# nep-pack/NonlinearEigenproblems.jl

Hardware: AMD Instinct MI355X
Metric: eigenpairs/sec (gun SPMF iar m=100) + compute_Mlincomb GB/s (higher is better)
Workload: dtype f64 (complex128)

## Files before the change

include/nepmi355.h:

```cpp
#ifndef NEPMI355_H
#define NEPMI355_H

#include <stddef.h>
#include <stdint.h>

#ifdef __cplusplus
extern "C" {
#endif

typedef struct { double re, im; } nep_cdouble;
typedef struct nep_spmf nep_spmf;
typedef struct nep_lu nep_lu;
typedef struct nep_comm nep_comm;
typedef void* nep_stream;

#define NEP_OK 0
#define NEP_ERR_HIP -1
#define NEP_ERR_ARG -2
#define NEP_ERR_SINGULAR -3
#define NEP_ERR_BREAKDOWN -4
#define NEP_ERR_UNSUPPORTED -5
#define NEP_ERR_RETRY -6
#define NEP_ERR_NOCONV -7

// ... 260 lines not shown
                                      nep_stream stream);

int32_t nep_devprim_exclusive_sum(const uint64_t* d_in, uint64_t* d_out, int64_t n, nep_stream stream);
int32_t nep_devprim_sort_pairs(uint64_t* d_keys, uint64_t* d_vals, int64_t n, int32_t nbits, nep_stream stream);

typedef struct nep_iar nep_iar;
int32_t nep_iar_create(nep_spmf* spmf, nep_lu* lu, int64_t n, int32_t m, nep_cdouble* dV, int64_t ldv,
                       const nep_cdouble* dCtab, int64_t ldc, const int64_t* d_active, nep_cdouble* dwork3n,
                       const double* h_cabs, const nep_cdouble* h_cf, int32_t mt, nep_cdouble* dH, nep_cdouble* h_pinnedH,
                       int32_t orth_method, nep_iar** out);
int32_t nep_iar_destroy(nep_iar* s);
int32_t nep_iar_step(nep_iar* s, int32_t k, int32_t refine_steps, nep_stream stream);
int32_t nep_iar_steps(nep_iar* s, int32_t k0, int32_t count, int32_t refine_steps, nep_stream stream);
int32_t nep_iar_wait(nep_iar* s, int32_t k);
int32_t nep_iar_stream_wait(nep_iar* s, int32_t k, nep_stream stream);

int32_t nep_basis_rotate(nep_cdouble* dV, int64_t ldv, int64_t rows, int32_t m, int32_t p, const nep_cdouble* hQ, int64_t ldq,
                         int32_t carry, nep_stream stream);

typedef struct nep_arnoldi nep_arnoldi;
int32_t nep_arnoldi_create(nep_spmf* spmf, nep_lu* lu, int64_t n, int32_t maxdim, nep_cdouble* dV, int64_t ldv,
                           const nep_cdouble* d_cB, nep_cdouble* dwork_n, nep_cdouble* dS, nep_cdouble* h_pinnedS,
                           int32_t orth_method, nep_arnoldi** out);
int32_t nep_arnoldi_destroy(nep_arnoldi* s);
int32_t nep_arnoldi_steps(nep_arnoldi* s, int32_t j0, int32_t count, nep_stream stream);
int32_t nep_arnoldi_wait(nep_arnoldi* s, int32_t j);

typedef struct nep_iar_opts {
    int32_t maxit;
    int32_t check_error_every;
// ... 8 lines not shown
typedef struct nep_iar_result {
    int32_t k;
    int32_t nconv;
    int32_t nret;
    int32_t refine_plan;
    int32_t refine_hint_off;
    int32_t retry_reason;
} nep_iar_result;
typedef int32_t (*nep_fv_eval)(void* ctx, int32_t nlam, const nep_cdouble* lam, nep_cdouble* F);
int32_t nep_refine_review(int32_t umfpack_refinements, int32_t plan, int32_t final_recorded, const double* w4, int32_t hint_in,
                          int32_t out[4]);
int32_t nep_iar_run(nep_spmf* spmf, nep_lu* lu, int64_t n, const nep_iar_opts* opts, const nep_cdouble* h_v0,
                    const nep_cdouble* h_Ctab, int32_t mt, const double* h_cabs, const nep_cdouble* h_cf, const double* h_fro,
                    nep_fv_eval fv, void* ctx, nep_cdouble* h_lam, nep_cdouble* dQ, nep_cdouble* h_Q, double* h_err,
                    nep_cdouble* dV_basis, nep_iar_result* res, nep_stream stream);

int32_t nep_comm_unique_id(void* h_out128);
int32_t nep_comm_create(int32_t rank, int32_t world, const void* h_unique_id128, nep_comm** out);
int32_t nep_comm_destroy(nep_comm* c);
int32_t nep_comm_info(const nep_comm* c, int32_t out[2]);
int32_t nep_allgather_sum(nep_comm* c, const nep_cdouble* d_partial, int64_t len, nep_cdouble* d_total, nep_stream stream);
int32_t nep_sum_ranks(const nep_cdouble* d_parts, int64_t len, int32_t world, nep_cdouble* d_total, nep_stream stream);

typedef struct nep_bem nep_bem;
int32_t nep_bem_create(int64_t n, const double* h_vert, const double* h_area, int32_t gauss_order, nep_bem** out);
int32_t nep_bem_destroy(nep_bem* b);
int32_t nep_bem_info(const nep_bem* b, int64_t info[4]);
int32_t nep_bem_static(const nep_bem* b, double* d_out, int64_t ldo, nep_stream stream);
int32_t nep_bem_assemble(const nep_bem* b, int32_t nlam, const nep_cdouble* h_lam, int32_t der, nep_cdouble* dOut, int64_t ldo,
                         int64_t stride, nep_stream stream);
// ... 20 lines not shown
```

nonlineareigenproblems.jl_amd/_lib.py:

```python
import ctypes as C
import os

import numpy as np
import torch

from ._env import env_flag

_HERE = os.path.dirname(os.path.abspath(__file__))
LIB_PATH = os.path.join(_HERE, "libnepmi355.so")


class NepError(RuntimeError):
    def __init__(self, status, msg):
        super().__init__("libnepmi355 status %d: %s" % (status, msg))
        self.status = status


NEP_OK, NEP_ERR_HIP, NEP_ERR_ARG, NEP_ERR_SINGULAR, NEP_ERR_BREAKDOWN, NEP_ERR_UNSUPPORTED = 0, -1, -2, -3, -4, -5
NEP_ERR_RETRY, NEP_ERR_NOCONV = -6, -7


def _load():
    from . import build
    if build.needs_build():
# ... 140 lines not shown
    "nep_iar_create": [c_vp, c_vp, c_i64, c_i32, c_vp, c_i64, c_vp, c_i64, c_vp, c_vp, c_vp, c_vp, c_i32, c_vp, c_vp, c_i32, P(c_vp)],
    "nep_iar_destroy": [c_vp],
    "nep_lu_refac_create": [c_vp, c_i64, c_vp, c_vp, c_vp, c_vp, c_vp, c_vp, c_vp, c_vp, c_vp],
    "nep_lu_refac_destroy": [c_vp],
    "nep_lu_refac_info": [c_vp, c_vp],
    "nep_lu_refac_wide_info": [c_vp, c_vp],
    "nep_lu_refac_hash": [c_vp, c_vp],
    "nep_lu_factor_dev": [c_vp, c_vp, c_i32, C.c_double, c_vp, c_vp, c_vp, c_vp],
    "nep_lu_refac_analyze": [c_i64, c_vp, c_vp, c_vp, c_vp, c_vp, c_vp, c_vp, c_vp, c_vp],
    "nep_lu_factor_dev_batch": [c_vp, c_i32, c_vp, c_i32, C.c_double, c_vp, c_vp, c_vp, c_vp],
    "nep_lu_factor_dev_batch_terms": [c_vp, c_i32, c_vp, c_i32, c_vp, c_i32, C.c_double, c_vp, c_vp, c_vp],
    "nep_iar_step": [c_vp, c_i32, c_i32, c_vp],
    "nep_iar_steps": [c_vp, c_i32, c_i32, c_i32, c_vp],
    "nep_iar_wait": [c_vp, c_i32],
    "nep_iar_stream_wait": [c_vp, c_i32, c_vp],
    "nep_basis_rotate": [c_vp, c_i64, c_i64, c_i32, c_i32, c_vp, c_i64, c_i32, c_vp],
    "nep_arnoldi_create": [c_vp, c_vp, c_i64, c_i32, c_vp, c_i64, c_vp, c_vp, c_vp, c_vp, c_i32, P(c_vp)],
    "nep_arnoldi_destroy": [c_vp],
    "nep_arnoldi_steps": [c_vp, c_i32, c_i32, c_vp],
    "nep_arnoldi_wait": [c_vp, c_i32],
    "nep_devprim_exclusive_sum": [c_vp, c_vp, c_i64, c_vp],
    "nep_devprim_sort_pairs": [c_vp, c_vp, c_i64, c_i32, c_vp],
    "nep_refine_review": [c_i32, c_i32, c_i32, c_vp, c_i32, c_vp],
    "nep_iar_run": [c_vp, c_vp, c_i64, c_vp, c_vp, c_vp, c_i32, c_vp, c_vp, c_vp, c_vp, c_vp, c_vp, c_vp, c_vp, c_vp, c_vp, c_vp, c_vp],
    "nep_hess_eig_worksize": [c_i32, P(c_i64)],
    "nep_hess_eigvals_dev": [c_i32, c_vp, c_i64, c_vp, c_vp, c_vp, c_vp],
    "nep_hess_eigvecs_dev": [c_i32, c_vp, c_vp, c_i64, c_vp, c_vp, c_vp],
    "nep_hess_eigvals_batch_dev": [c_i32, c_i32, c_i32, c_vp, c_i64, c_vp, c_i64, c_vp, c_i64, c_vp, c_i64, c_vp],
    "nep_hess_eigvecs_batch_dev": [c_i32, c_i32, c_i32, c_vp, c_i64, c_vp, c_i64, c_i64, c_vp, c_i64, c_vp, c_i64, c_vp],
    "nep_comm_unique_id": [c_vp],
    "nep_comm_create": [c_i32, c_i32, c_vp, P(c_vp)],
    "nep_comm_destroy": [c_vp],
    "nep_comm_info": [c_vp, P(c_i32)],
    "nep_allgather_sum": [c_vp, c_vp, c_i64, c_vp, c_vp],
    "nep_sum_ranks": [c_vp, c_i64, c_i32, c_vp, c_vp],
    "nep_iar_shift_scale": [c_i64, c_i32, c_vp, c_vp, c_vp],
    "nep_rk_bw": [c_i64, c_i32, c_vp, c_vp, c_vp, c_vp],
    "nep_discretize_polygon": [c_i32, c_vp, c_i32, c_vp],
    "nep_block_recur": [c_i64, c_i32, c_vp, c_vp, c_vp, c_vp, c_vp],
# ... 59 lines not shown
```

nonlineareigenproblems.jl_amd/csrc/driver.hip:

```cpp
#include "common.h"
#include <vector>
#include <stdlib.h>
#include <time.h>

struct nep_iar {
    nep_spmf* spmf; nep_lu* lu;
    int64_t n, ldv; int32_t m, mt;
    cplx* dV; const cplx* dCtab; int64_t ldc; const int64_t* d_active;
    cplx* dz; cplx* dW;
    std::vector<double> cabs; std::vector<nep_cdouble> cf;
    cplx* dH; nep_cdouble* hH;
    double* d_cabs; cplx* d_ccf;
    cplx* hH_dev;
    int32_t method;
    std::vector<hipEvent_t> ev;
    hipEvent_t e_upload = nullptr; bool upload_waited = false;
    hipStream_t last = nullptr;
    bool no_events = false;
    std::vector<hipGraphExec_t> graphs;
    cplx* dWT = nullptr; int32_t wt_for = 0;
};

extern "C" {

int32_t nep_iar_create(nep_spmf* spmf, nep_lu* lu, int64_t n, int32_t m, nep_cdouble* dV, int64_t ldv,
                       const nep_cdouble* dCtab, int64_t ldc, const int64_t* d_active, nep_cdouble* dwork3n,
                       const double* h_cabs, const nep_cdouble* h_cf, int32_t mt, nep_cdouble* dH, nep_cdouble* h_pinnedH,
                       int32_t orth_method, nep_iar** out) {
    ARGCHK(out != nullptr);
    *out = nullptr;
    ARGCHK(spmf && lu && dV && dCtab && dwork3n && dH && h_pinnedH);
    ARGCHK(n > 0 && m >= 1 && ldv >= n * (int64_t)(m + 1) && ldc >= m && mt >= 1 && (orth_method == 0 || orth_method == 1));
    nep_iar* s = new nep_iar();
// ... 91 lines not shown
        rc = nep_iar_shift_scale(n, k, (const nep_cdouble*)col, (nep_cdouble*)vv, stream);
        if (rc) return rc;
    }
    cplx* mirror = s->hH_dev ? s->hH_dev + (int64_t)(k - 1) * (s->m + 4) : nullptr;
    if (s->dWT && k < s->m) {
        rc = nep_orth_dev_iar_next((const nep_cdouble*)s->dV, s->ldv, n, k, s->d_active, (nep_cdouble*)vv, (nep_cdouble*)hrow, s->method,
                                   (nep_cdouble*)mirror, k + 4, (const nep_cdouble*)s->dCtab, s->ldc, s->mt,
                                   (nep_cdouble*)s->dWT, (nep_cdouble*)(vv + s->ldv + n), stream);
        if (!rc) s->wt_for = k + 1;
    } else
        rc = nep_orth_dev_mirror((const nep_cdouble*)s->dV, s->ldv, n * (int64_t)(k + 1), k, s->d_active, (nep_cdouble*)vv,
                                 (nep_cdouble*)hrow, s->method, (nep_cdouble*)mirror, k + 4, stream);
    if (rc) return rc;
    if (!mirror)
        HIPCHK(hipMemcpyAsync(s->hH + (int64_t)(k - 1) * (s->m + 4), hrow, (size_t)(k + 4) * sizeof(cplx), hipMemcpyDeviceToHost, st));
    if (s->no_events) return NEP_OK;
    if (!s->ev[k]) HIPCHK(hipEventCreateWithFlags(&s->ev[k], hipEventDisableTiming | hipEventBlockingSync));
    HIPCHK(hipEventRecord(s->ev[k], st));
    return NEP_OK;
}

int32_t nep_iar_steps(nep_iar* s, int32_t k0, int32_t count, int32_t refine_steps, nep_stream stream) {
    ARGCHK(s && count >= 1);
    for (int32_t k = k0; k < k0 + count; ++k) {
        int rc = nep_iar_step(s, k, refine_steps, stream);
        if (rc) return rc;
    }
    return NEP_OK;
}

int32_t nep_iar_steps_graph(nep_iar* s, int32_t k0, int32_t count, int32_t refine_steps, nep_stream stream, int32_t* captured) {
    ARGCHK(s && count >= 1);
    if (captured) *captured = 0;
// ... 8 lines not shown
        hipGraph_t g = nullptr;
        hipError_t e = hipStreamEndCapture(st, &g);
        hipGraphExec_t ge = nullptr;
        if (!rc && e == hipSuccess && g && hipGraphInstantiate(&ge, g, nullptr, nullptr, 0) == hipSuccess && ge) {
            if (hipGraphLaunch(ge, st) == hipSuccess) { s->graphs.push_back(ge); ok = true; }
            else (void)hipGraphExecDestroy(ge);
        }
        if (g) (void)hipGraphDestroy(g);
        if (!ok) (void)hipGetLastError();
    } else (void)hipGetLastError();
    if (!ok) {
        s->wt_for = wt_for0; s->upload_waited = waited0; s->last = last0;
        return nep_iar_steps(s, k0, count, refine_steps, stream);
    }
    for (int32_t k = k0; k < k0 + count; ++k) {
        if (!s->ev[k]) HIPCHK(hipEventCreateWithFlags(&s->ev[k], hipEventDisableTiming | hipEventBlockingSync));
        HIPCHK(hipEventRecord(s->ev[k], st));
    }
    if (captured) *captured = 1;
    return NEP_OK;
}

int32_t nep_iar_wait(nep_iar* s, int32_t k) {
    ARGCHK(s && k >= 1 && k <= s->m && s->ev[k]);
    for (;;) {
        const hipError_t e = hipEventQuery(s->ev[k]);
        if (e == hipSuccess) return NEP_OK;
        if (e != hipErrorNotReady) HIPCHK(e);
        struct timespec ts = {0, 20000};
        nanosleep(&ts, nullptr);
    }
}

int32_t nep_iar_stream_wait(nep_iar* s, int32_t k, nep_stream stream) {
    ARGCHK(s && k >= 1 && k <= s->m && s->ev[k]);
    HIPCHK(hipStreamWaitEvent(as_stream(stream), s->ev[k], 0));
    return NEP_OK;
}

}
```

nonlineareigenproblems.jl_amd/csrc/iar_run.hip:

```cpp
#include "common.h"
#include <algorithm>
#include <deque>
#include <map>
#include <mutex>
#include <vector>
#include <math.h>
#include <time.h>

extern "C" {
int32_t nep_iar_create(nep_spmf* spmf, nep_lu* lu, int64_t n, int32_t m, nep_cdouble* dV, int64_t ldv, const nep_cdouble* dCtab,
                       int64_t ldc, const int64_t* d_active, nep_cdouble* dwork3n, const double* h_cabs, const nep_cdouble* h_cf,
                       int32_t mt, nep_cdouble* dH, nep_cdouble* h_pinnedH, int32_t orth_method, nep_iar** out);
int32_t nep_iar_steps_graph(nep_iar* s, int32_t k0, int32_t count, int32_t refine_steps, nep_stream stream, int32_t* captured);
}

namespace {

constexpr double EPS = 2.220446049250313e-16;

__global__ void k_iar_active(int64_t* act, int64_t n, int m1) {
    const int j = blockIdx.x * blockDim.x + threadIdx.x;
    if (j < m1) act[j] = (int64_t)(j + 1) * n;
}
__global__ void k_iar_start(cplx* __restrict__ V, const cplx* __restrict__ v, double inv, int64_t n) {
    const int64_t i = (int64_t)blockIdx.x * blockDim.x + threadIdx.x;
    if (i < n) V[i] = cmake(v[i].x * inv, v[i].y * inv);
}

constexpr int64_t ZSLACK = 8192;
__global__ __launch_bounds__(256) void k_iar_zero_slack(cplx* __restrict__ V, int64_t ldv, int64_t n, int m1) {
    const int j = blockIdx.y;
    const int64_t a = (int64_t)(j + 1) * n;
    const int64_t r = a + (int64_t)blockIdx.x * 256 + threadIdx.x;
// ... 160 lines not shown
    std::vector<hipEvent_t> ev_pool;
    std::vector<double> s_lam; std::vector<int> s_idx; cplx* s_QT = nullptr; int s_kq = 0; int conv = 0; int k_checked = 0;
    std::vector<double> s_err;
    double* h_err = nullptr;
    int retry = 0;

    hipEvent_t event() {
        if (!ev_pool.empty()) { hipEvent_t e = ev_pool.back(); ev_pool.pop_back(); return e; }
        hipEvent_t e = nullptr;
        if (hipEventCreateWithFlags(&e, hipEventDisableTiming) != hipSuccess) { (void)hipGetLastError(); return nullptr; }
        return e;
    }
    void done(hipEvent_t e) { if (e) ev_pool.push_back(e); }

    int fail_kind = 0, fail_at = 0;
    int fill_H(int kk) {
        for (int j = 1; j <= kk; ++j) {
            if (filled[j]) continue;
            if (fail_at == j && (fail_kind == 1 || fail_kind == 2)) {
                retry = fail_kind; nep_set_error("nep_iar_run: injected miss of kind %d at step %d", fail_kind, j); return NEP_ERR_RETRY;
            }
            const cplx* row = a.Hpin + (int64_t)(j - 1) * (m + 4);
            const int flags = (int)row[j + 1].y;
            if (flags & 2) { nep_set_error("orthogonalisation breakdown in step %d: ||w|| = %g", j, row[j].x); return NEP_ERR_BREAKDOWN; }
            if ((flags & 1) && o.orth_method == 0) { retry = 2; nep_set_error("nep_iar_run: step %d wanted another DGKS pass", j); return NEP_ERR_RETRY; }
            if (ref.umf > 0) {
                const int plan = plans[j];
                const bool final_rec = !((plan & 0x100) && (j % 8) != 0);
                if (!ref.review((const double*)(row + j + 2), plan & 0xff, final_rec)) {
                    retry = 1; nep_set_error("nep_iar_run: the refinement record of step %d asks for more sweeps than were taken", j);
                    return NEP_ERR_RETRY;
                }
            }
            filled[j] = 1;
        }
        return NEP_OK;
    }
    ~Run() {
        if (step) (void)nep_iar_destroy(step);
        if (V && own_V) nep_pool_free_on(V, st, true);
        if (s_QT) nep_pool_free_on(s_QT, rs.check, true);
        for (hipEvent_t e : ev_pool) (void)hipEventDestroy(e);
        if (have_arena) arena_return(a);
    }
};

}

extern "C" {

int32_t nep_refine_review(int32_t umfpack_refinements, int32_t plan, int32_t final_recorded, const double* w4, int32_t hint_in,
                          int32_t out[4]) {
    ARGCHK(w4 && out && plan >= 0 && plan <= 3 && umfpack_refinements >= 0);
    Refine r; r.umf = umfpack_refinements; r.hint = hint_in;
    const bool ok = r.review(w4, plan, final_recorded != 0);
    out[0] = ok ? 1 : 0; out[1] = r.recorded; out[2] = r.hint; out[3] = r.hint_off ? 1 : 0;
    return NEP_OK;
}

int32_t nep_iar_run(nep_spmf* spmf, nep_lu* lu, int64_t n, const nep_iar_opts* opts, const nep_cdouble* h_v0,
                    const nep_cdouble* h_Ctab, int32_t mt, const double* h_cabs, const nep_cdouble* h_cf, const double* h_fro,
                    nep_fv_eval fv, void* ctx, nep_cdouble* h_lam, nep_cdouble* dQ, nep_cdouble* h_Q, double* h_err,
                    nep_cdouble* dV_basis, nep_iar_result* res, nep_stream stream) {
    ARGCHK(spmf && lu && opts && h_v0 && h_Ctab && fv && h_lam && res);
    ARGCHK(n > 0 && mt >= 1 && opts->maxit >= 1 && opts->check_error_every >= 1);
    ARGCHK(opts->orth_method == 0 || opts->orth_method == 1);
    ARGCHK(opts->errmeasure == 0 || (opts->errmeasure == 1 && h_fro));
    ARGCHK(opts->umfpack_refinements <= 0 || (h_cabs && h_cf));
    memset(res, 0, sizeof(*res));
    res->refine_plan = -1;
    struct timespec t_e_; clock_gettime(CLOCK_MONOTONIC, &t_e_);
    const double t_entry = t_e_.tv_sec * 1e3 + t_e_.tv_nsec * 1e-6;
    const int32_t m = opts->maxit;
    if (m > 128) { nep_set_error("nep_iar_run: maxit = %d exceeds the device eigen-decomposition's limit 128", m); return NEP_ERR_UNSUPPORTED; }
    const int BMAX = std::max(1, nep_env_int("NEP_IAR_EIG_BATCH", 16));
    const int LASTB = std::max(1, nep_env_int("NEP_IAR_EIG_LAST", 8));
    const double T100 = nep_env_double("NEP_IAR_EIG_MS100", 3.3);
    const double TSTEP = 0.35;
    const int cee = opts->check_error_every;
    const double neigs = opts->neigs;
    const bool unthrottled = isinf(neigs) && neigs > 0;

    Run R; R.spmf = spmf; R.lu = lu; R.n = n; R.o = *opts; R.fv = fv; R.ctx = ctx; R.h_fro = h_fro; R.st = as_stream(stream);
    R.m = m; R.mt = mt; R.ldv = n * (int64_t)(m + 1); R.h_err = h_err;
    int rc = run_streams(R.st, &R.rs); if (rc) return rc;
    rc = arena_acquire(n, m, mt, BMAX, &R.a); if (rc) return rc;
    R.have_arena = true;
    Arena& a = R.a;
    hipStream_t st = R.st, cst = R.rs.check, est = R.rs.eig;
    R.ref.umf = opts->umfpack_refinements > 0 ? opts->umfpack_refinements : 0;
    R.ref.hint = (opts->refine_hint >= 0 && nep_env_int("NEP_REFINE_HINT", 1) != 0) ? opts->refine_hint : -1;
    R.filled.assign(m + 1, 0); R.plans.assign(m + 1, 0);
    if (const char* fa = getenv("NEP_IAR_RUN_FAIL_AT")) { if (sscanf(fa, "%d:%d", &R.fail_kind, &R.fail_at) != 2) R.fail_kind = R.fail_at = 0; }
    if (h_err) for (int64_t i = 0; i < (int64_t)m * m; ++i) h_err[i] = NAN;

    if (dV_basis) { R.V = (cplx*)dV_basis; R.own_V = false; }
// ... 14 lines not shown
    }
    hipLaunchKernelGGL(k_iar_start, dim3((unsigned)((n + 255) / 256)), dim3(256), 0, st, R.V, (const cplx*)a.v0, 1.0 / sqrt(nrm2), n);
    hipLaunchKernelGGL(k_iar_active, dim3((unsigned)((m + 1 + 63) / 64)), dim3(64), 0, st, a.active, n, m + 1);
    HIPCHK(hipMemsetAsync(a.Hdev, 0, (size_t)m * (m + 4) * 16, st));
    LAUNCHCHK();
    memset(a.Hpin, 0, (size_t)m * (m + 4) * 16);
    memset(a.wpin, 0, (size_t)m * (m + 2) * 16);
    {
        static thread_local PinnedRing ring;
        rc = ring.upload(a.Ctab, h_Ctab, (size_t)m * mt * 16, st); if (rc) return rc;
    }
    rc = nep_iar_create(spmf, lu, n, m, (nep_cdouble*)R.V, R.ldv, (const nep_cdouble*)a.Ctab, m, a.active, (nep_cdouble*)a.work3n,
                        R.ref.umf > 0 ? h_cabs : nullptr, R.ref.umf > 0 ? h_cf : nullptr, mt, (nep_cdouble*)a.Hdev,
                        (nep_cdouble*)a.Hpin, opts->orth_method, &R.step);
    if (rc) return rc;

    std::vector<char> plan_end(m + 2, 0);
    if (unthrottled) {
        std::vector<int> allk;
        for (int kk = 1; kk <= m; ++kk) if (kk % cee == 0 || kk == m) allk.push_back(kk);
        int e_ = (int)allk.size(); int size = std::min(LASTB, e_);
        while (e_ > 0) {
            plan_end[allk[e_ - 1]] = 1; e_ -= size;
            if (e_ > 0) {
                const double q = allk[e_ - 1] / 100.0;
                size = (int)std::min<double>(std::min(BMAX, e_), std::max(1.0, ceil(2.0 * T100 * q * q / (TSTEP * cee))));
            }
        }
    }
    const bool trace = getenv("NEP_IAR_RUN_TRACE") != nullptr;
    auto now = []() { struct timespec t; clock_gettime(CLOCK_MONOTONIC, &t); return t.tv_sec * 1e3 + t.tv_nsec * 1e-6; };
    double t_fv = 0;
    std::deque<int> pendA; std::deque<Batch> stA; std::deque<Check> stC;
    int slots = unthrottled ? m + 1 : std::max(BMAX, 4);
    const int CHUNK = unthrottled ? 8 : 4;
    const int P = std::min(256, std::max(1, 3072 / mt));
    int k = 1; bool done = false; int status = NEP_OK;
    const bool use_graph = nep_env_flag("NEP_IAR_GRAPH");
    int n_graph = 0;
    auto finished = [&]() { return R.conv >= neigs; };

    auto batch_ready = [&]() -> int {
        if (pendA.empty()) return 0;
        int cnt = 1;
        while (cnt < (int)pendA.size() && cnt < BMAX && pendA[cnt] - pendA[cnt - 1] == pendA[1] - pendA[0] && !(unthrottled && plan_end[pendA[cnt - 1]])) ++cnt;
        if (!unthrottled || plan_end[pendA[cnt - 1]] || cnt >= BMAX || done) return cnt;
        return 0;
    };
    auto launch_batch = [&](int count) -> int {
        Batch b;
        for (int i = 0; i < count; ++i) { b.kcs.push_back(pendA.front()); pendA.pop_front(); }
        const int k0 = b.kcs[0], nb = count; b.kmax = b.kcs.back();
        const int kstep = nb > 1 ? b.kcs[1] - k0 : 0;
        int r = nep_iar_stream_wait(R.step, b.kmax, (nep_stream)est); if (r) return r;
        cplx* wrow = a.wdev + (int64_t)(k0 - 1) * (m + 2);
        cplx* mrow = a.wpin + (int64_t)(k0 - 1) * (m + 2);
        r = nep_hess_eigvals_batch_dev(nb, k0, kstep, (const nep_cdouble*)a.Hdev, m + 4, (nep_cdouble*)wrow, (int64_t)kstep * (m + 2),
                                       a.eigwork, a.wsz, (nep_cdouble*)mrow, (int64_t)kstep * (m + 2), (nep_stream)est);
        if (r) return r;
        b.evW = R.event(); if (!b.evW) return NEP_ERR_HIP;
        HIPCHK(hipEventRecord(b.evW, est));
        void* pz = nullptr;
        r = nep_pool_alloc(&pz, (size_t)nb * b.kmax * b.kmax * 16); if (r) return r;
        b.Zb = (cplx*)pz;
        r = nep_hess_eigvecs_batch_dev(nb, k0, kstep, (nep_cdouble*)wrow, (int64_t)kstep * (m + 2), (nep_cdouble*)b.Zb, b.kmax,
                                       (int64_t)b.kmax * b.kmax, a.eigwork, a.wsz, (nep_cdouble*)mrow, (int64_t)kstep * (m + 2), (nep_stream)est);
        if (r) { nep_pool_free_on(b.Zb, est, true); return r; }
        b.evZ = R.event(); if (!b.evZ) return NEP_ERR_HIP;
        HIPCHK(hipEventRecord(b.evZ, est));
        stA.push_back(b);
        return NEP_OK;
    };
    auto launch_check = [&](const Batch& b, int bi, bool first_of_batch) -> int {
        const int kc = b.kcs[bi];
        int r = R.fill_H(kc); if (r) return r;
        const cplx* w = a.wpin + (int64_t)(kc - 1) * (m + 2);
        if (w[kc].x != 0.0 || (R.fail_kind == 3 && R.fail_at == kc)) { R.retry = 3; nep_set_error("nep_iar_run: the QR iteration of step %d gave up", kc); return NEP_ERR_RETRY; }
        Check c; c.kc = kc; c.lam.resize(2 * (size_t)kc); c.F.resize(2 * (size_t)mt * kc);
        const double sr = R.o.sigma.re, si = R.o.sigma.im, gr = R.o.gamma.re, gi = R.o.gamma.im;
        for (int s = 0; s < kc; ++s) {
            const double dr = w[s].x, di = w[s].y, den = dr * dr + di * di;
            c.lam[2 * s] = sr + (gr * dr + gi * di) / den;
            c.lam[2 * s + 1] = si + (gi * dr - gr * di) / den;
        }
        const double tf0 = trace ? now() : 0.0;
        const int32_t frc = R.fv(R.ctx, kc, (const nep_cdouble*)c.lam.data(), (nep_cdouble*)c.F.data());
        if (trace) t_fv += now() - tf0;
        if (frc != 0) {
            nep_set_error("nep_iar_run: the f_t(lambda) callback failed in step %d", kc); return NEP_ERR_ARG;
        }
        if (first_of_batch) HIPCHK(hipStreamWaitEvent(cst, b.evZ, 0));
        void* pq = nullptr;
        r = nep_pool_alloc(&pq, (size_t)n * kc * 16); if (r) return r;
        c.QT = (cplx*)pq;
        r = nep_gemm_ts_dev((const nep_cdouble*)R.V, R.ldv, n, kc, (const nep_cdouble*)(b.Zb + (int64_t)bi * b.kmax * b.kmax), b.kmax, 0, kc,
                            (nep_cdouble*)c.QT, kc, 1, (nep_stream)cst);
        double* d_out = a.d_norms + (int64_t)(kc - 1) * 2 * m;
        if (!r) r = nep_resid_batch_dev(spmf, kc, (const nep_cdouble*)c.F.data(), (const nep_cdouble*)c.QT, kc, d_out, (nep_stream)cst);
        if (r) { nep_pool_free_on(c.QT, cst, true); return r; }
        HIPCHK(hipMemcpyAsync(a.npin + (int64_t)(kc - 1) * 2 * m, d_out, (size_t)2 * kc * 8, hipMemcpyDeviceToHost, cst));
        c.ev = R.event(); if (!c.ev) return NEP_ERR_HIP;
        HIPCHK(hipEventRecord(c.ev, cst));
        if (bi == (int)b.kcs.size() - 1) c.Zb_owner = b.Zb;
        stC.push_back(std::move(c));
        return NEP_OK;
    };
// ... 42 lines not shown
        return NEP_OK;
    };
    auto drop_check = [&](Check& c) {
        if (c.QT) nep_pool_free_on(c.QT, cst, true);
        if (c.Zb_owner) nep_pool_free_on(c.Zb_owner, cst, true);
        R.done(c.ev);
    };
    auto drop_batch = [&](Batch& b) {
        if (b.Zb) nep_pool_free_on(b.Zb, est, true);
        R.done(b.evW); R.done(b.evZ);
    };

    hipEvent_t te0 = nullptr, te1 = nullptr; bool te1_rec = false;
    if (trace) { (void)hipEventCreate(&te0); (void)hipEventCreate(&te1); (void)hipEventRecord(te0, st); }
    const double t_loop = now();
    double tt_steps = 0, tt_A = 0, tt_B = 0, tt_C = 0, tt_sleep = 0, t_enq_done = 0; double tq = 0;
    while (status == NEP_OK) {
        bool progressed = false;
        tq = now();
        if (!done) {
            if (k <= m && !finished()) {
                int nb = 0;
                while (nb < CHUNK && k + nb <= m) {
                    const bool due = ((k + nb) % cee == 0) || (k + nb == m);
                    if (due) { if (slots <= 0) break; --slots; }
                    ++nb;
                }
                if (nb > 0) {
                    int plan = R.ref.plan();
                    if (plan > 0 && R.ref.settled()) plan |= 0x100;
                    if (use_graph && k > 1) { int32_t cap = 0; status = nep_iar_steps_graph(R.step, k, nb, plan, stream, &cap); n_graph += cap; }
                    else status = nep_iar_steps(R.step, k, nb, plan, stream);
                    if (status) break;
                    for (int kk = k; kk < k + nb; ++kk) {
                        R.plans[kk] = plan;
                        if (kk % cee == 0 || kk == m) pendA.push_back(kk);
                    }
                    k += nb; progressed = true;
                }
            } else done = true;
            if (k > m) { if (!done && trace) { t_enq_done = now() - t_loop; if (te1 && !te1_rec) { (void)hipEventRecord(te1, st); te1_rec = true; } } done = true; }
        }
        if (trace) { const double t = now(); tt_steps += t - tq; tq = t; }
        while (!finished()) {
            const int cnt = batch_ready();
            if (!cnt) break;
            status = launch_batch(cnt); progressed = true;
            if (status) break;
        }
        if (status) break;
        if (trace) { const double t = now(); tt_A += t - tq; tq = t; }
        while (!stA.empty() && !finished() && ev_done(stA.front().evW)) {
            progressed = true;
            Batch b = stA.front(); stA.pop_front();
            for (int bi = 0; bi < (int)b.kcs.size() && status == NEP_OK; ++bi) {
                status = launch_check(b, bi, bi == 0);
// ... 22 lines not shown
        if (done && pendA.empty() && stA.empty() && stC.empty()) break;
        if (!progressed) { struct timespec ts = {0, 20000}; nanosleep(&ts, nullptr); if (trace) { const double t = now(); tt_sleep += t - tq; tq = t; } }
    }
    if (trace)
        fprintf(stderr, "nep_iar_run trace (ms): set-up %.2f | loop %.2f: steps %.2f (all enqueued at %.2f) A %.2f B %.2f (callback %.2f) C %.2f sleep %.2f\n",
                t_loop - t_entry, now() - t_loop, tt_steps, t_enq_done, tt_A, tt_B, t_fv, tt_C, tt_sleep);
    if (trace && use_graph) fprintf(stderr, "nep_iar_run: %d chunks went out as hipGraphs\n", n_graph);
    if (trace && te0 && te1 && te1_rec) {
        float ms_ = 0.0f;
        if (hipEventSynchronize(te1) == hipSuccess && hipEventElapsedTime(&ms_, te0, te1) == hipSuccess)
            fprintf(stderr, "nep_iar_run: the recurrence's %d steps took %.2f ms on the device\n", m, ms_);
        (void)hipGetLastError();
    }
    if (te0) (void)hipEventDestroy(te0);
    if (te1) (void)hipEventDestroy(te1);
    while (!stA.empty()) { drop_batch(stA.front()); stA.pop_front(); }
    while (!stC.empty()) { drop_check(stC.front()); stC.pop_front(); }
    (void)hipStreamSynchronize(est);
    (void)hipStreamSynchronize(cst);
    res->retry_reason = R.retry;
    res->refine_plan = R.ref.hint_off ? -1 : (R.ref.recorded >= 0 ? R.ref.recorded : R.ref.hint);
    res->refine_hint_off = R.ref.hint_off ? 1 : 0;
    if (status || !unthrottled) (void)hipStreamSynchronize(st);
    if (status) return status;

    int nret = (int)(R.s_lam.size() / 2);
    const bool noconv = (R.conv < neigs) && !unthrottled;
    if (!noconv) nret = std::min(nret, R.conv);
    res->k = R.k_checked > 0 ? R.k_checked : k - 1;
    res->nconv = R.conv; res->nret = nret;
    for (int s = 0; s < nret; ++s) { h_lam[s].re = R.s_lam[2 * s]; h_lam[s].im = R.s_lam[2 * s + 1]; }
    if (nret > 0 && (dQ || h_Q) && R.s_QT) {
        cplx* dst = (cplx*)dQ; void* tmp = nullptr;
        if (!dst) { rc = nep_pool_alloc(&tmp, (size_t)n * nret * 16); if (rc) return rc; dst = (cplx*)tmp; }
        std::vector<int32_t> cols(R.s_idx.begin(), R.s_idx.begin() + nret);
        rc = nep_rowmajor_to_colmajor(n, R.s_kq, (const nep_cdouble*)R.s_QT, R.s_kq, cols.data(), nret, (nep_cdouble*)dst, n, (nep_stream)cst);
        if (!rc && h_Q) {
            if (hipMemcpyAsync(h_Q, dst, (size_t)n * nret * 16, hipMemcpyDeviceToHost, cst) != hipSuccess) rc = NEP_ERR_HIP;
        }
        if (hipStreamSynchronize(cst) != hipSuccess && !rc) rc = NEP_ERR_HIP;
        if (tmp) nep_pool_free(tmp);
        if (rc) { if (rc == NEP_ERR_HIP) nep_set_error("nep_iar_run: returning the eigenvector block failed"); return rc; }
    }
    if (noconv) { nep_set_error("Number of iterations exceeded. maxit=%d.", m); return NEP_ERR_NOCONV; }
    return NEP_OK;
}

}
```

nonlineareigenproblems.jl_amd/iar.py:

```python
import contextlib
import ctypes as _C
import queue
import threading
import time
from collections import deque
from concurrent.futures import ThreadPoolExecutor
from typing import NamedTuple

import numpy as np
import torch

from . import dense, _hosteig
from ._affinity import cpu_budget
from ._env import env_flag, env_float, env_int, env_str
from ._lib import (lib, check, c_vp, c_i32, hptr, cdouble, NepError, IarOpts, IarResult, FV_EVAL, NEP_ERR_BREAKDOWN, NEP_ERR_RETRY,
                   NEP_ERR_NOCONV)
from ._ritzchecks import RitzChecks
from ._streams import _check_stream, _eig_streams
from .errmeasure import (DefaultErrmeasure, ResidualErrmeasure, StandardSPMFErrmeasure, estimate_errors, estimate_errors_async)
from .exceptions import NoConvergenceException
from .linsolvers import DefaultLinSolverCreator, FactorizeLinSolver, create_linsolver
from .nep import CDT, AbstractSPMF, pure_spmf, to_host, to_host_cm, stream_ptr

EPS = np.finfo(float).eps
# ... 116 lines not shown

def _route(f):
    if not f.staged():
        return "sync"
    if not f.native():
        return "async"
    dev_eig = f.m <= dense.HESS_EIG_KMAX and env_str("NEP_IAR_EIG", "dev") != "host"
    if (f.native_run and f.native_err and dev_eig and env_str("NEP_IAR_NATIVE_RUN", "1") != "0"
            and not any(env_flag(e) for e in ("NEP_IAR_TRACE", "NEP_IAR_ONE_STREAM", "NEP_IAR_PASSES"))):
        return "run"
    if env_flag("NEP_IAR_ONE_STREAM") or not f.batch_async:
        return "async"
    return "step+deveig" if dev_eig else "step+hosteig"


def _iar_native_run(nep, M0inv, orthmethod, m, tol, neigs, errkind, sigma, gamma, v, check_error_every, errhist, return_device):
    n = nep.size(1)
    fv = nep.get_fv(); mt = len(fv)
    alpha = gamma ** np.arange(m + 1); alpha[0] = 0
    tab = nep.derivative_table(sigma, m)
    Ctab = np.asfortranarray((alpha[1:m + 1] / np.arange(1, m + 1))[:, None] * tab["fD"][1:m + 1, :], dtype=np.complex128)
    v0 = np.ascontiguousarray(v, dtype=np.complex128)
    rc_ = M0inv.refine_coefficients() if M0inv.umfpack_refinements > 0 else None
    if M0inv.umfpack_refinements > 0 and rc_ is None:
        return None
    o = IarOpts(m, int(check_error_every), dense._orth_code(orthmethod), int(max(0, M0inv.umfpack_refinements)), errkind[0],
                -1, float(tol), float(neigs), cdouble(sigma.real, sigma.imag), cdouble(gamma.real, gamma.imag))
    res = IarResult()

    def fv_eval(ctx, nlam, lam_p, F_p):
        try:
            la = np.frombuffer((_C.c_double * (2 * nlam)).from_address(lam_p), dtype=np.complex128)
            F = np.frombuffer((_C.c_double * (2 * nlam * mt)).from_address(F_p), dtype=np.complex128).reshape(nlam, mt)
            for t, f in enumerate(fv):
                F[:, t] = f.values(la)
            return 0
        except Exception:
            import traceback
            traceback.print_exc()
            return 1
    cb = FV_EVAL(fv_eval)
    ldv = n * (m + 1)
    V = torch.empty((m + 1, ldv), dtype=CDT, device="cuda")
    Qd = torch.empty((m, n), dtype=CDT, device="cuda") if return_device else None
    Qh = None if return_device else torch.empty((m, n), dtype=CDT, pin_memory=True)
    lam = np.zeros(m, dtype=np.complex128)
    err = np.full((m, m), np.nan, order="F")
    st = M0inv.refine.native_run(o, res, lambda: lib.nep_iar_run(
        nep.dev.h, M0inv.lu.h, n, _C.addressof(o), hptr(v0), hptr(Ctab), mt,
        hptr(rc_[0]) if rc_ else None, hptr(rc_[1]) if rc_ else None, hptr(errkind[1]) if errkind[1] is not None else None,
        _C.cast(cb, c_vp), None, hptr(lam), c_vp(Qd.data_ptr()) if Qd is not None else None,
        c_vp(Qh.data_ptr()) if Qh is not None else None, hptr(err), c_vp(V.data_ptr()), _C.addressof(res), stream_ptr()))
    if st == NEP_ERR_RETRY:
        if res.retry_reason == 1:
            raise _RefinementMiss(0)
        if res.retry_reason == 2:
            raise _OrthPassMiss(0)
        raise _NativeRunMiss(res.retry_reason)
    if st not in (0, NEP_ERR_NOCONV):
        check(st)
    iar.native_runs += 1
    iar.last_route = "run"
    k = int(res.k); nret = int(res.nret)
    M0inv.refine.solves += k
    if errhist is not None:
        for kc in range(1, k + 1):
            if kc % check_error_every == 0 or kc == m:
# ... 19 lines not shown
        linsolvercreator = DefaultLinSolverCreator()
    if errmeasure is None:
        errmeasure = DefaultErrmeasure(nep)
    if v is None:
        v = np.random.randn(n)
    errkind = _native_errmeasure(errmeasure, nep)
    f = _Facts(m=m, orth=dense._orth_code(orthmethod), dev_lu=True, native_err=errkind is not None,
               spmf_dev=_plain_spmf(nep) and type(nep).resid_norms is AbstractSPMF.resid_norms and hasattr(nep, "dev"),
               batch_async=hasattr(errmeasure, "batch_async"), timed=timers is not None, proj_solve=bool(proj_solve),
               native_run=_native_run, native_step=_native_step, force_sync=_force_sync)
    M0inv = None
    if _route(f) == "run":
        M0inv = create_linsolver(linsolvercreator, nep, sigma)
        if _device_lu(M0inv):
            out = _iar_native_run(nep, M0inv, orthmethod, m, tol, neigs, errkind, sigma, gamma, v, check_error_every, errhist,
                                  return_device)
            if out is not None:
                return out
    s = _State(t_entry, nep, orthmethod, m, linsolvercreator, M0inv, tol, neigs, errmeasure, sigma, gamma, v, check_error_every,
               proj_solve, errhist, timers, inner_solver_method, f.staged())
    f = f._replace(native_run=False, spmf_dev=_plain_spmf(nep) and "Cdev" in s.tab, dev_lu=_device_lu(s.M0inv))
    if f.native() and not s.create_native_step():
        f = f._replace(dev_lu=False)
    route = iar.last_route = _route(f)
    s.start(route)
    try:
        k = {"sync": _run_sync, "async": _run_async}.get(route, _run_steps)(s)
    finally:
        s.close()
    k = s.checks.k_checked if s.checks.k_checked > 0 else k - 1
    lam, Q = s.checks.finish(k, maxit, "Try to change the inner_solver_method for better performance.",
# ... 489 lines not shown
```

Before: 1434.

## Skip per-step error history and thin IAR events when unthrottled without history

When neigs is infinite and no error history or logger is requested, the native IAR run sets the check cadence to the final step only. It also records completion events only at chunk boundaries, and the host no longer allocates the error matrix. Row review and refinement checks are decoupled from the eigenvalue checks and done lazily: a lag gate polls step readiness with a non-blocking query before enqueuing further chunks, and the rest is reviewed once enqueueing finishes. The aim is to cut Hessenberg eigen decompositions, residual checks, event records and host syncs, at the cost of more complex control flow and bounded enqueue-ahead.

```diff
diff --git a/include/nepmi355.h b/include/nepmi355.h
--- a/include/nepmi355.h
+++ b/include/nepmi355.h
@@ -298,6 +298,8 @@
 int32_t nep_iar_steps(nep_iar* s, int32_t k0, int32_t count, int32_t refine_steps, nep_stream stream);
 int32_t nep_iar_wait(nep_iar* s, int32_t k);
 int32_t nep_iar_stream_wait(nep_iar* s, int32_t k, nep_stream stream);
+int32_t nep_iar_ready(nep_iar* s, int32_t k, int32_t* ready);
+int32_t nep_iar_event_mask(nep_iar* s, const uint8_t* mask);
 
 int32_t nep_basis_rotate(nep_cdouble* dV, int64_t ldv, int64_t rows, int32_t m, int32_t p, const nep_cdouble* hQ, int64_t ldq,
                          int32_t carry, nep_stream stream);
@@ -336,6 +338,7 @@
                     const nep_cdouble* h_Ctab, int32_t mt, const double* h_cabs, const nep_cdouble* h_cf, const double* h_fro,
                     nep_fv_eval fv, void* ctx, nep_cdouble* h_lam, nep_cdouble* dQ, nep_cdouble* h_Q, double* h_err,
                     nep_cdouble* dV_basis, nep_iar_result* res, nep_stream stream);
+int32_t nep_iar_run_stats(int32_t out[4]);
 
 int32_t nep_comm_unique_id(void* h_out128);
 int32_t nep_comm_create(int32_t rank, int32_t world, const void* h_unique_id128, nep_comm** out);
diff --git a/nonlineareigenproblems.jl_amd/_lib.py b/nonlineareigenproblems.jl_amd/_lib.py
--- a/nonlineareigenproblems.jl_amd/_lib.py
+++ b/nonlineareigenproblems.jl_amd/_lib.py
@@ -178,6 +178,8 @@
     "nep_iar_steps": [c_vp, c_i32, c_i32, c_i32, c_vp],
     "nep_iar_wait": [c_vp, c_i32],
     "nep_iar_stream_wait": [c_vp, c_i32, c_vp],
+    "nep_iar_ready": [c_vp, c_i32, P(c_i32)],
+    "nep_iar_event_mask": [c_vp, c_vp],
     "nep_basis_rotate": [c_vp, c_i64, c_i64, c_i32, c_i32, c_vp, c_i64, c_i32, c_vp],
     "nep_arnoldi_create": [c_vp, c_vp, c_i64, c_i32, c_vp, c_i64, c_vp, c_vp, c_vp, c_vp, c_i32, P(c_vp)],
     "nep_arnoldi_destroy": [c_vp],
@@ -187,6 +189,7 @@
     "nep_devprim_sort_pairs": [c_vp, c_vp, c_i64, c_i32, c_vp],
     "nep_refine_review": [c_i32, c_i32, c_i32, c_vp, c_i32, c_vp],
     "nep_iar_run": [c_vp, c_vp, c_i64, c_vp, c_vp, c_vp, c_i32, c_vp, c_vp, c_vp, c_vp, c_vp, c_vp, c_vp, c_vp, c_vp, c_vp, c_vp, c_vp],
+    "nep_iar_run_stats": [P(c_i32)],
     "nep_hess_eig_worksize": [c_i32, P(c_i64)],
     "nep_hess_eigvals_dev": [c_i32, c_vp, c_i64, c_vp, c_vp, c_vp, c_vp],
     "nep_hess_eigvecs_dev": [c_i32, c_vp, c_vp, c_i64, c_vp, c_vp, c_vp],
diff --git a/nonlineareigenproblems.jl_amd/csrc/driver.hip b/nonlineareigenproblems.jl_amd/csrc/driver.hip
--- a/nonlineareigenproblems.jl_amd/csrc/driver.hip
+++ b/nonlineareigenproblems.jl_amd/csrc/driver.hip
@@ -17,6 +17,8 @@
     hipEvent_t e_upload = nullptr; bool upload_waited = false;
     hipStream_t last = nullptr;
     bool no_events = false;
+    std::vector<uint8_t> ev_mask;
+    int32_t n_ev = 0;
     std::vector<hipGraphExec_t> graphs;
     cplx* dWT = nullptr; int32_t wt_for = 0;
 };
@@ -138,9 +140,23 @@
     if (rc) return rc;
     if (!mirror)
         HIPCHK(hipMemcpyAsync(s->hH + (int64_t)(k - 1) * (s->m + 4), hrow, (size_t)(k + 4) * sizeof(cplx), hipMemcpyDeviceToHost, st));
-    if (s->no_events) return NEP_OK;
+    if (s->no_events || (!s->ev_mask.empty() && !s->ev_mask[k])) return NEP_OK;
     if (!s->ev[k]) HIPCHK(hipEventCreateWithFlags(&s->ev[k], hipEventDisableTiming | hipEventBlockingSync));
     HIPCHK(hipEventRecord(s->ev[k], st));
+    ++s->n_ev;
+    return NEP_OK;
+}
+
+int32_t nep_iar_event_mask(nep_iar* s, const uint8_t* mask) {
+    ARGCHK(s != nullptr);
+    ARGCHK(s->last == nullptr && s->n_ev == 0);
+    if (mask) s->ev_mask.assign(mask, mask + s->m + 1); else s->ev_mask.clear();
+    return NEP_OK;
+}
+
+int32_t nep_iar_events_recorded(const nep_iar* s, int32_t* out) {
+    ARGCHK(s && out);
+    *out = s->n_ev;
     return NEP_OK;
 }
 
@@ -179,8 +195,10 @@
         return nep_iar_steps(s, k0, count, refine_steps, stream);
     }
     for (int32_t k = k0; k < k0 + count; ++k) {
+        if (!s->ev_mask.empty() && !s->ev_mask[k]) continue;
         if (!s->ev[k]) HIPCHK(hipEventCreateWithFlags(&s->ev[k], hipEventDisableTiming | hipEventBlockingSync));
         HIPCHK(hipEventRecord(s->ev[k], st));
+        ++s->n_ev;
     }
     if (captured) *captured = 1;
     return NEP_OK;
@@ -197,6 +215,15 @@
     }
 }
 
+int32_t nep_iar_ready(nep_iar* s, int32_t k, int32_t* ready) {
+    ARGCHK(s && ready && k >= 1 && k <= s->m && s->ev[k]);
+    const hipError_t e = hipEventQuery(s->ev[k]);
+    if (e == hipErrorNotReady) (void)hipGetLastError();
+    else if (e != hipSuccess) HIPCHK(e);
+    *ready = e == hipSuccess ? 1 : 0;
+    return NEP_OK;
+}
+
 int32_t nep_iar_stream_wait(nep_iar* s, int32_t k, nep_stream stream) {
     ARGCHK(s && k >= 1 && k <= s->m && s->ev[k]);
     HIPCHK(hipStreamWaitEvent(as_stream(stream), s->ev[k], 0));
diff --git a/nonlineareigenproblems.jl_amd/csrc/iar_run.hip b/nonlineareigenproblems.jl_amd/csrc/iar_run.hip
--- a/nonlineareigenproblems.jl_amd/csrc/iar_run.hip
+++ b/nonlineareigenproblems.jl_amd/csrc/iar_run.hip
@@ -12,11 +12,14 @@
                        int64_t ldc, const int64_t* d_active, nep_cdouble* dwork3n, const double* h_cabs, const nep_cdouble* h_cf,
                        int32_t mt, nep_cdouble* dH, nep_cdouble* h_pinnedH, int32_t orth_method, nep_iar** out);
 int32_t nep_iar_steps_graph(nep_iar* s, int32_t k0, int32_t count, int32_t refine_steps, nep_stream stream, int32_t* captured);
+int32_t nep_iar_events_recorded(const nep_iar* s, int32_t* out);
 }
 
 namespace {
 
 constexpr double EPS = 2.220446049250313e-16;
+
+thread_local int32_t g_run_stats[4] = {0, 0, 0, 0};
 
 __global__ void k_iar_active(int64_t* act, int64_t n, int m1) {
     const int j = blockIdx.x * blockDim.x + threadIdx.x;
@@ -207,16 +210,28 @@
     void done(hipEvent_t e) { if (e) ev_pool.push_back(e); }
 
     int fail_kind = 0, fail_at = 0;
-    int fill_H(int kk) {
-        for (int j = 1; j <= kk; ++j) {
-            if (filled[j]) continue;
-            if (fail_at == j && (fail_kind == 1 || fail_kind == 2)) {
+    int flagged = 0, reviewed = 0;
+    int check_flags(int kk) {
+        for (int j = flagged + 1; j <= kk; ++j) {
+            if (fail_at == j && fail_kind == 2) {
                 retry = fail_kind; nep_set_error("nep_iar_run: injected miss of kind %d at step %d", fail_kind, j); return NEP_ERR_RETRY;
             }
             const cplx* row = a.Hpin + (int64_t)(j - 1) * (m + 4);
             const int flags = (int)row[j + 1].y;
             if (flags & 2) { nep_set_error("orthogonalisation breakdown in step %d: ||w|| = %g", j, row[j].x); return NEP_ERR_BREAKDOWN; }
             if ((flags & 1) && o.orth_method == 0) { retry = 2; nep_set_error("nep_iar_run: step %d wanted another DGKS pass", j); return NEP_ERR_RETRY; }
+            flagged = j;
+        }
+        return NEP_OK;
+    }
+    int fill_H(int kk) {
+        const int rf = check_flags(kk); if (rf) return rf;
+        for (int j = 1; j <= kk; ++j) {
+            if (filled[j]) continue;
+            if (fail_at == j && fail_kind == 1) {
+                retry = fail_kind; nep_set_error("nep_iar_run: injected miss of kind %d at step %d", fail_kind, j); return NEP_ERR_RETRY;
+            }
+            const cplx* row = a.Hpin + (int64_t)(j - 1) * (m + 4);
             if (ref.umf > 0) {
                 const int plan = plans[j];
                 const bool final_rec = !((plan & 0x100) && (j % 8) != 0);
@@ -225,12 +240,13 @@
                     return NEP_ERR_RETRY;
                 }
             }
-            filled[j] = 1;
-        }
+            filled[j] = 1; ++g_run_stats[3];
+        }
+        reviewed = std::max(reviewed, kk);
         return NEP_OK;
     }
     ~Run() {
-        if (step) (void)nep_iar_destroy(step);
+        if (step) { (void)nep_iar_events_recorded(step, &g_run_stats[2]); (void)nep_iar_destroy(step); }
         if (V && own_V) nep_pool_free_on(V, st, true);
         if (s_QT) nep_pool_free_on(s_QT, rs.check, true);
         for (hipEvent_t e : ev_pool) (void)hipEventDestroy(e);
@@ -255,6 +271,7 @@
                     const nep_cdouble* h_Ctab, int32_t mt, const double* h_cabs, const nep_cdouble* h_cf, const double* h_fro,
                     nep_fv_eval fv, void* ctx, nep_cdouble* h_lam, nep_cdouble* dQ, nep_cdouble* h_Q, double* h_err,
                     nep_cdouble* dV_basis, nep_iar_result* res, nep_stream stream) {
+    for (int i = 0; i < 4; ++i) g_run_stats[i] = 0;
     ARGCHK(spmf && lu && opts && h_v0 && h_Ctab && fv && h_lam && res);
     ARGCHK(n > 0 && mt >= 1 && opts->maxit >= 1 && opts->check_error_every >= 1);
     ARGCHK(opts->orth_method == 0 || opts->orth_method == 1);
@@ -270,9 +287,13 @@
     const int LASTB = std::max(1, nep_env_int("NEP_IAR_EIG_LAST", 8));
     const double T100 = nep_env_double("NEP_IAR_EIG_MS100", 3.3);
     const double TSTEP = 0.35;
-    const int cee = opts->check_error_every;
     const double neigs = opts->neigs;
     const bool unthrottled = isinf(neigs) && neigs > 0;
+    const bool nohist = unthrottled && !h_err;
+    const int cee = nohist ? m : opts->check_error_every;
+    auto due_at = [&](int kk) { return kk % cee == 0 || kk == m; };
+    const int CHUNK = unthrottled ? 8 : 4;
+    const int LAG = 3 * CHUNK;
 
     Run R; R.spmf = spmf; R.lu = lu; R.n = n; R.o = *opts; R.fv = fv; R.ctx = ctx; R.h_fro = h_fro; R.st = as_stream(stream);
     R.m = m; R.mt = mt; R.ldv = n * (int64_t)(m + 1); R.h_err = h_err;
@@ -317,11 +338,16 @@
                         R.ref.umf > 0 ? h_cabs : nullptr, R.ref.umf > 0 ? h_cf : nullptr, mt, (nep_cdouble*)a.Hdev,
                         (nep_cdouble*)a.Hpin, opts->orth_method, &R.step);
     if (rc) return rc;
+    if (nohist) {
+        std::vector<uint8_t> mask(m + 1, 0);
+        for (int kk = 1; kk <= m; ++kk) mask[kk] = (kk % CHUNK == 0 || kk == m) ? 1 : 0;
+        rc = nep_iar_event_mask(R.step, mask.data()); if (rc) return rc;
+    }
 
     std::vector<char> plan_end(m + 2, 0);
     if (unthrottled) {
         std::vector<int> allk;
-        for (int kk = 1; kk <= m; ++kk) if (kk % cee == 0 || kk == m) allk.push_back(kk);
+        for (int kk = 1; kk <= m; ++kk) if (due_at(kk)) allk.push_back(kk);
         int e_ = (int)allk.size(); int size = std::min(LASTB, e_);
         while (e_ > 0) {
             plan_end[allk[e_ - 1]] = 1; e_ -= size;
@@ -336,7 +362,6 @@
     double t_fv = 0;
     std::deque<int> pendA; std::deque<Batch> stA; std::deque<Check> stC;
     int slots = unthrottled ? m + 1 : std::max(BMAX, 4);
-    const int CHUNK = unthrottled ? 8 : 4;
     const int P = std::min(256, std::max(1, 3072 / mt));
     int k = 1; bool done = false; int status = NEP_OK;
     const bool use_graph = nep_env_flag("NEP_IAR_GRAPH");
@@ -361,6 +386,7 @@
         r = nep_hess_eigvals_batch_dev(nb, k0, kstep, (const nep_cdouble*)a.Hdev, m + 4, (nep_cdouble*)wrow, (int64_t)kstep * (m + 2),
                                        a.eigwork, a.wsz, (nep_cdouble*)mrow, (int64_t)kstep * (m + 2), (nep_stream)est);
         if (r) return r;
+        g_run_stats[0] += nb;
         b.evW = R.event(); if (!b.evW) return NEP_ERR_HIP;
         HIPCHK(hipEventRecord(b.evW, est));
         void* pz = nullptr;
@@ -376,7 +402,7 @@
     };
     auto launch_check = [&](const Batch& b, int bi, bool first_of_batch) -> int {
         const int kc = b.kcs[bi];
-        int r = R.fill_H(kc); if (r) return r;
+        int r = R.check_flags(kc); if (r) return r;
         const cplx* w = a.wpin + (int64_t)(kc - 1) * (m + 2);
         if (w[kc].x != 0.0 || (R.fail_kind == 3 && R.fail_at == kc)) { R.retry = 3; nep_set_error("nep_iar_run: the QR iteration of step %d gave up", kc); return NEP_ERR_RETRY; }
         Check c; c.kc = kc; c.lam.resize(2 * (size_t)kc); c.F.resize(2 * (size_t)mt * kc);
@@ -393,6 +419,7 @@
             nep_set_error("nep_iar_run: the f_t(lambda) callback failed in step %d", kc); return NEP_ERR_ARG;
         }
         if (first_of_batch) HIPCHK(hipStreamWaitEvent(cst, b.evZ, 0));
+        ++g_run_stats[1];
         void* pq = nullptr;
         r = nep_pool_alloc(&pq, (size_t)n * kc * 16); if (r) return r;
         c.QT = (cplx*)pq;
@@ -465,16 +492,23 @@
     hipEvent_t te0 = nullptr, te1 = nullptr; bool te1_rec = false;
     if (trace) { (void)hipEventCreate(&te0); (void)hipEventCreate(&te1); (void)hipEventRecord(te0, st); }
     const double t_loop = now();
-    double tt_steps = 0, tt_A = 0, tt_B = 0, tt_C = 0, tt_sleep = 0, t_enq_done = 0; double tq = 0;
+    double tt_steps = 0, tt_A = 0, tt_B = 0, tt_C = 0, tt_sleep = 0, t_enq_done = 0, t_m_done = 0; double tq = 0;
     while (status == NEP_OK) {
         bool progressed = false;
         tq = now();
         if (!done) {
             if (k <= m && !finished()) {
+                const int g = (k - 1) / CHUNK * CHUNK - LAG;
+                bool gate_open = true;
+                if (g >= 1 && !R.filled[g]) {
+                    int32_t ready = 0;
+                    status = nep_iar_ready(R.step, g, &ready); if (status) break;
+                    if (ready) { status = R.fill_H(g); if (status) break; }
+                    else gate_open = false;
+                }
                 int nb = 0;
-                while (nb < CHUNK && k + nb <= m) {
-                    const bool due = ((k + nb) % cee == 0) || (k + nb == m);
-                    if (due) { if (slots <= 0) break; --slots; }
+                while (gate_open && nb < CHUNK && k + nb <= m && !(nb > 0 && (k + nb - 1) % CHUNK == 0)) {
+                    if (due_at(k + nb)) { if (slots <= 0) break; --slots; }
                     ++nb;
                 }
                 if (nb > 0) {
@@ -485,12 +519,23 @@
                     if (status) break;
                     for (int kk = k; kk < k + nb; ++kk) {
                         R.plans[kk] = plan;
-                        if (kk % cee == 0 || kk == m) pendA.push_back(kk);
+                        if (due_at(kk)) pendA.push_back(kk);
                     }
                     k += nb; progressed = true;
                 }
             } else done = true;
             if (k > m) { if (!done && trace) { t_enq_done = now() - t_loop; if (te1 && !te1_rec) { (void)hipEventRecord(te1, st); te1_rec = true; } } done = true; }
+        }
+        if (k > m && !finished()) {
+            while (R.reviewed < m) {
+                const int g = std::min((R.reviewed / CHUNK + 1) * CHUNK, m);
+                int32_t ready = 0;
+                status = nep_iar_ready(R.step, g, &ready); if (status || !ready) break;
+                status = R.fill_H(g); if (status) break;
+                progressed = true;
+                if (g == m && trace) t_m_done = now();
+            }
+            if (status) break;
         }
         if (trace) { const double t = now(); tt_steps += t - tq; tq = t; }
         while (!finished()) {
@@ -543,6 +588,7 @@
     }
     if (te0) (void)hipEventDestroy(te0);
     if (te1) (void)hipEventDestroy(te1);
+    if (status == NEP_OK && R.k_checked > 0) status = R.fill_H(R.k_checked);
     while (!stA.empty()) { drop_batch(stA.front()); stA.pop_front(); }
     while (!stC.empty()) { drop_check(stC.front()); stC.pop_front(); }
     (void)hipStreamSynchronize(est);
@@ -571,8 +617,17 @@
         if (tmp) nep_pool_free(tmp);
         if (rc) { if (rc == NEP_ERR_HIP) nep_set_error("nep_iar_run: returning the eigenvector block failed"); return rc; }
     }
+    if (trace && t_m_done > 0)
+        fprintf(stderr, "nep_iar_run: %.2f ms from the arrival of step %d's row to the return (%d decompositions, %d checks)\n",
+                now() - t_m_done, m, g_run_stats[0], g_run_stats[1]);
     if (noconv) { nep_set_error("Number of iterations exceeded. maxit=%d.", m); return NEP_ERR_NOCONV; }
     return NEP_OK;
 }
 
-}
+int32_t nep_iar_run_stats(int32_t out[4]) {
+    ARGCHK(out != nullptr);
+    for (int i = 0; i < 4; ++i) out[i] = g_run_stats[i];
+    return NEP_OK;
+}
+
+}
diff --git a/nonlineareigenproblems.jl_amd/iar.py b/nonlineareigenproblems.jl_amd/iar.py
--- a/nonlineareigenproblems.jl_amd/iar.py
+++ b/nonlineareigenproblems.jl_amd/iar.py
@@ -154,7 +154,12 @@
     return "step+deveig" if dev_eig else "step+hosteig"
 
 
-def _iar_native_run(nep, M0inv, orthmethod, m, tol, neigs, errkind, sigma, gamma, v, check_error_every, errhist, return_device):
+def _native_run_keeps_history(errhist, neigs, logger):
+    return errhist is not None or bool(logger) or not (np.isinf(neigs) and neigs > 0)
+
+
+def _iar_native_run(nep, M0inv, orthmethod, m, tol, neigs, errkind, sigma, gamma, v, check_error_every, errhist, return_device,
+                    logger=0):
     n = nep.size(1)
     fv = nep.get_fv(); mt = len(fv)
     alpha = gamma ** np.arange(m + 1); alpha[0] = 0
@@ -185,12 +190,13 @@
     Qd = torch.empty((m, n), dtype=CDT, device="cuda") if return_device else None
     Qh = None if return_device else torch.empty((m, n), dtype=CDT, pin_memory=True)
     lam = np.zeros(m, dtype=np.complex128)
-    err = np.full((m, m), np.nan, order="F")
+    err = np.full((m, m), np.nan, order="F") if _native_run_keeps_history(errhist, neigs, logger) else None
     st = M0inv.refine.native_run(o, res, lambda: lib.nep_iar_run(
         nep.dev.h, M0inv.lu.h, n, _C.addressof(o), hptr(v0), hptr(Ctab), mt,
         hptr(rc_[0]) if rc_ else None, hptr(rc_[1]) if rc_ else None, hptr(errkind[1]) if errkind[1] is not None else None,
         _C.cast(cb, c_vp), None, hptr(lam), c_vp(Qd.data_ptr()) if Qd is not None else None,
-        c_vp(Qh.data_ptr()) if Qh is not None else None, hptr(err), c_vp(V.data_ptr()), _C.addressof(res), stream_ptr()))
+        c_vp(Qh.data_ptr()) if Qh is not None else None, hptr(err) if err is not None else None, c_vp(V.data_ptr()),
+        _C.addressof(res), stream_ptr()))
     if st == NEP_ERR_RETRY:
         if res.retry_reason == 1:
             raise _RefinementMiss(0)
@@ -240,7 +246,7 @@
         M0inv = create_linsolver(linsolvercreator, nep, sigma)
         if _device_lu(M0inv):
             out = _iar_native_run(nep, M0inv, orthmethod, m, tol, neigs, errkind, sigma, gamma, v, check_error_every, errhist,
-                                  return_device)
+                                  return_device, logger)
             if out is not None:
                 return out
     s = _State(t_entry, nep, orthmethod, m, linsolvercreator, M0inv, tol, neigs, errmeasure, sigma, gamma, v, check_error_every,
```

Measured after the change: 1580, median of 6. +10.2%, better.
